# nkb-tech/nkb-classification

Measured on AMD Instinct MI355X. Metric: images/sec train step (3x224x224), higher is better.
Workload: dtype bf16; 1 GPU; resnet50 single-task train step, 1000 classes, bs=256/GPU, bf16 compute + fp32 master weights, NAdam, 3x224x224; global_batch=256, parallelism=dp1

## Files before the change

include/nkbhip.h:

```cpp
#ifndef NKBHIP_H
#define NKBHIP_H
#include <stddef.h>
#ifdef __cplusplus
extern "C" {
#endif

typedef struct ihipStream_t* nkb_stream_t;

#define NKB_DT_F32 0
#define NKB_DT_BF16 1
#define NKB_ACT_GELU 0
#define NKB_ACT_QUICK_GELU 1

const char* nkb_last_error(void);
int nkb_version(void);
enum NkbLaunchCounter {
    NKB_LAUNCH_GEMM8P = 0,
    NKB_LAUNCH_WGRAD8P = 1,
    NKB_LAUNCH_WGRAD3X3 = 2,
    NKB_LAUNCH_WGRAD8F = 3,
    NKB_LAUNCH_GRAM_CONV = 4,
    NKB_LAUNCH_GRAM_BN_APPLY = 5,
    NKB_LAUNCH_CONVP = 6,
    NKB_LAUNCH_CONV1P = 7,
// ... 81 lines not shown
                          void* g_masked, const void* c_prev, const float* scale, const float* shift, const float* mean, float* stats,
                          long long M, int Cout, int ldy, nkb_stream_t stream);
int nkb_gram_fold2(int dtype, const void* w1, const float* s1, int K1, const void* w2, const float* s2, int K2, int Cout, void* out,
                   const float* shift1, const float* shift2, float* shift_out, nkb_stream_t stream);
int nkb_conv_cat_relu_bits(int dtype, const void* a, int lda, int K1, const void* x, int ldx, int K2, const void* wf, const float* shift,
                           void* y, unsigned char* relu_bits, long long M, int Cout, int ldy, nkb_stream_t stream);
int nkb_conv_cat_bias(int dtype, const void* a, int lda, int K1, const void* x, int ldx, int K2, const void* w, const float* bias, void* y,
                      long long M, int Cout, int ldy, nkb_stream_t stream);
int nkb_conv_dgrad_bn_cat(int dtype, const void* g, int ldg, int K1, const void* a, int lda, int K2, const void* wcat,
                          const float* cbias, void* g_masked, const void* c_prev, const float* scale, const float* shift,
                          const float* mean, float* stats, long long M, int Cout, int ldy, nkb_stream_t stream);
size_t nkb_bn_backward_workspace_floats(long long rows, int C);

int nkb_maxpool3x3s2(int dtype, int backward, const void* in, void* out, unsigned char* idx, int N, int H, int W, int C,
                     nkb_stream_t stream);
enum NkbPoolMode {
    NKB_POOL_AVG_FWD = 0,
    NKB_POOL_AVG_BWD = 1,
    NKB_GRN_FWD_REDUCE = 2,
    NKB_GRN_FWD_APPLY = 3,
    NKB_GRN_BWD_REDUCE = 4,
    NKB_GRN_BWD_APPLY = 5,
    NKB_GRN_PARAM = 6
};
enum NkbSeMode {
    NKB_SE_POOL = 16,
    NKB_SE_GATE = 17,
    NKB_ECA_GATE = 18,
    NKB_SE_FWD_APPLY = 19,
    NKB_SE_BWD_REDUCE = 20,
    NKB_SE_BWD_GATE = 21,
    NKB_ECA_BWD_GATE = 22,
    NKB_SE_BWD_APPLY = 23
};
int nkb_avgpool(int dtype, int mode, const void* in, void* out, int N, int HW, int C, const void* in2, const float* weight,
                const float* bias, float* sumsq, float* dweight, float* dbias, const void* mul, float eps, float* workspace,
                long long workspace_floats, nkb_stream_t stream);
int nkb_bn_relu_maxpool(int dtype, int backward, const void* c, const float* scale, const float* shift,
                        const float* mean, const float* invstd, const float* gamma, void* y_or_g, unsigned char* idx,
                        void* dc, float* dgamma, float* dbeta, float* workspace, size_t workspace_floats, int N, int H,
                        int W, int C, nkb_stream_t stream);
int nkb_bn_relu_maxpool_sel(int dtype, int backward, const void* c, const float* scale, const float* shift,
                            const float* mean, const float* invstd, const float* gamma, void* y_or_g, unsigned char* idx,
                            void* dc, float* dgamma, float* dbeta, float* workspace, size_t workspace_floats, void* xsel,
                            int N, int H, int W, int C, nkb_stream_t stream);
size_t nkb_bn_relu_maxpool_workspace_floats(int N, int H, int W, int C);

int nkb_im2row(int dtype, const float* x, void* col, int N, int Cin, int H, int W, int R, int S, int stride, int pad,
               int Kp, nkb_stream_t stream);

int nkb_stem_pack(int dtype, const float* x, void* out, int N, int C, int H, int W, nkb_stream_t stream);
int nkb_stem_wprep(int dtype, const float* w, void* wp, int Cout, int C, nkb_stream_t stream);
int nkb_stem_weight_cols(int dtype);
int nkb_stem_conv(int dtype, const void* xp, const void* wp, void* y, float* stats, int N, int H, int W, int Cout,
                  int ldy, nkb_stream_t stream);
long long nkb_gramr_workspace_floats(int dtype, long long M, int co, int ci);
int nkb_gramr(int dtype, const void* g, int ldg, const void* a, int lda, float* R, long long M, int co, int ci, int mode,
              float* workspace, long long workspace_floats, nkb_stream_t stream);
int nkb_stemp_tiles(int dtype, int N, int H, int W, int Cout);
long long nkb_stemp_wgrad_workspace_floats(int dtype, int N, int H, int W, int Cout);
int nkb_stemp_wgrad(int dtype, const void* dy, const void* xp, float* dwp, int N, int H, int W, int Cout, int lddy, float* workspace,
                    long long workspace_floats, nkb_stream_t stream);
int nkb_stemp_conv(int dtype, const void* xp, const void* wp, void* y, float* stats, int N, int H, int W, int Cout, int ldy,
                   nkb_stream_t stream);
int nkb_stem_wgrad(int dtype, const void* dy, const void* xp, float* dwp, int N, int H, int W, int Cout, int lddy,
                   float* workspace, long long workspace_floats, nkb_stream_t stream);
// ... 133 lines not shown
```

nkb-classification_amd/csrc/conv_igemm.hip:

```cpp
#include "common.h"
#include "prims.h"
#include <type_traits>

#include "conv_params.h"
#include "wgrad256.h"
#include "gemm8p.h"
#include "wgrad3x3.h"
#include "wgradr.h"


template <typename T> struct MmaTraits;
template <> struct MmaTraits<bf16_t> { static constexpr int KSTEPS = 2; };
template <> struct MmaTraits<float> { static constexpr int KSTEPS = 8; };

constexpr int EPI_GENERAL = 0, EPI_BN_MASK = 1, EPI_BN_BITS = 2, EPI_LEAN = 3, EPI_AFFINE_BITS = 4, EPI_BN_BITS_LEAN = 6,
              EPI_BN_MASK_LEAN = 7, EPI_LEAN_CAT = 8;
template <typename T, int TC, int TP, int BNB = 0, bool HALO = false>
__global__ __launch_bounds__(256, ((BNB && TC == 128) || TC == 64) ? 3 : 1) void conv_igemm_kernel(const ConvParams p) {
    constexpr int EPC = DT<T>::EPC;
    constexpr int KTE = 128 / (int)sizeof(T);
    constexpr int NWR = TC / 32;
    constexpr int NPR = TP / 32;
    constexpr int MC = TC / 32;
    constexpr int MP = TP / 32;
    constexpr int NPX = HALO ? (TP + 2 + 31) / 32 : NPR;
    constexpr int STAGE_BYTES = (TC + 32 * NPX) * 128;
    constexpr int EROW = TC * 4 + 16;
    extern __shared__ __attribute__((aligned(16))) unsigned char smem[];

    const int tid = threadIdx.x;
    const int lane = tid & 63;
    const int wave = tid >> 6;
    const int wc = wave >> 1, wp = wave & 1;

    const unsigned nwg = gridDim.x;
// ... 1129 lines not shown
            return launch_conv_impl<T, TC, TP, BNB, true>(p, stream, batch);
    }
    return launch_conv_impl<T, TC, TP, BNB, false>(p, stream, batch);
}
static bool narrow_tile(int Cout) { return Cout <= 64; }
template <int BNB>
static int launch_conv(ConvParams& p, int dtype, bool narrow, hipStream_t stream, int batch = 1) {
    if constexpr (BNB != EPI_AFFINE_BITS && BNB != EPI_LEAN_CAT) {
        if (dtype != NKB_DT_BF16)
            return narrow ? launch_conv_tile<float, 64, 256, BNB>(p, stream, batch) : launch_conv_tile<float, 128, 128, BNB>(p, stream, batch);
    }
    if constexpr (BNB != EPI_AFFINE_BITS) {
        if (narrow) return launch_conv_tile<bf16_t, 64, 256, BNB>(p, stream, batch);
    }
    return launch_conv_tile<bf16_t, 128, 128, BNB>(p, stream, batch);
}

static ConvParams conv_geometry(int N, int H, int W, int Cin, int ldx, int P, int Q, int Cout, int ldy, int R, int S, int stride, int pad,
                                int mode) {
    ConvParams p;
    p.M = N * P * Q; p.H = H; p.W = W; p.Cin = Cin; p.ldx = ldx; p.P = P; p.Q = Q; p.Cout = Cout; p.ldy = ldy;
    p.R = R; p.S = S; p.stride = stride; p.pad = pad; p.mode = mode;
    p.stride_w = stride; p.pad_w = pad;
    p.divPQ = make_fastdiv((unsigned)(P * Q)); p.divQ = make_fastdiv((unsigned)Q);
    p.ldw = R * S * Cin;
    return p;
}
static ConvParams gemm_geometry(int M, int K, int N, int ldx, int ldw, int ldy) {
    ConvParams p = conv_geometry(1, M, 1, K, ldx, M, 1, N, ldy, 1, 1, 1, 0, 0);
    p.ldw = ldw;
    return p;
}

extern "C" int nkb_conv_gemm(int dtype, int mode, const void* x, const void* w, void* y, const void* add,
                             const float* bias, float* stats, int N, int H, int W, int Cin, int ldx, int P, int Q,
                             int Cout, int ldy, int ldadd, int R, int S, int stride, int pad, int relu, int out_f32,
                             int add_h, int add_w, const unsigned char* add_bits, hipStream_t stream) {
    const int esz = dtype == NKB_DT_BF16 ? 2 : 4;
    const int kte = 128 / esz;
    if (dtype != NKB_DT_BF16 && dtype != NKB_DT_F32) { nkb_set_error("conv_gemm: bad dtype %d", dtype); return 1; }
    if (Cin % kte != 0 || ldx % (16 / esz) != 0) {
        nkb_set_error("conv_gemm: Cin=%d must be a multiple of %d and ldx=%d of %d", Cin, kte, ldx, 16 / esz);
        return 1;
    }
    if (stride != 1 && stride != 2) { nkb_set_error("conv_gemm: stride %d unsupported", stride); return 1; }
    if (R > 32 || S > 32) { nkb_set_error("conv_gemm: %dx%d filter exceeds the 32-tap-per-axis validity masks", R, S); return 1; }
    if ((long long)N * H * W * ldx * esz >= 0xFFFFFF00ll || (long long)Cout * R * S * Cin * esz >= 0xFFFFFF00ll) {
        nkb_set_error("conv_gemm: operand exceeds the 4 GiB buffer-addressing range");
        return 1;
    }
    if ((long long)N * H * W * ldx >= (1ll << 31) || (long long)N * P * Q * ldy >= (1ll << 31) ||
        (long long)Cout * R * S * Cin >= (1ll << 31)) {
        nkb_set_error("conv_gemm: tensor exceeds 2^31 elements");
        return 1;
    }
    if (add_bits && (add == nullptr || add_h > 0 || ldadd % 8 != 0)) { nkb_set_error("conv_gemm: add_bits needs a full-grid add with ldadd %% 8 == 0"); return 1; }
    ConvParams p = conv_geometry(N, H, W, Cin, ldx, P, Q, Cout, ldy, R, S, stride, pad, mode);
    p.x = x; p.w = w; p.y = y; p.add = add; p.bias = bias; p.stats = stats;
    p.ldadd = ldadd; p.relu = relu; p.out_f32 = out_f32;
    p.add_h = add_h; p.add_w = add_w; p.add_bits = add_bits;
    const double flops = 2.0 * p.M * (double)Cout * R * S * Cin;
    const double bytes = ((double)N * H * W * Cin + (double)Cout * R * S * Cin) * esz +
                         (double)p.M * Cout * (out_f32 ? 4 : esz) * (add ? 2 : 1);
    NkbProfScope prof(mode == 0 ? NKB_K_CONV_FWD : NKB_K_CONV_DGRAD, stream, flops, bytes);
    if (nkb_gemm8p_eligible(p, dtype, 1)) return nkb_launch_gemm8p(p, stream);
    return launch_conv<EPI_GENERAL>(p, dtype, narrow_tile(Cout), stream);
}

extern "C" int nkb_conv_dgrad_bn(int dtype, const void* dy, const void* w, void* g_masked, const void* c,
                                 const float* scale, const float* shift, const float* mean, float* stats,
                                 const unsigned char* relu_bits, const void* add, int ldadd, const unsigned char* add_bits,
                                 int add_h, int add_w, int N, int H,
                                 int W, int Cin, int ldx, int P, int Q, int Cout, int ldy, int R, int S, int stride, int pad,
                                 hipStream_t stream) {
    const int esz = dtype == NKB_DT_BF16 ? 2 : 4;
    const int kte = 128 / esz;
    if (dtype != NKB_DT_BF16 && dtype != NKB_DT_F32) { nkb_set_error("conv_dgrad_bn: bad dtype %d", dtype); return 1; }
    if (Cin % kte != 0 || ldx % (16 / esz) != 0 || Cout % 8 != 0 || ldy % 8 != 0) {
        nkb_set_error("conv_dgrad_bn: Cin=%d must be a multiple of %d, Cout=%d / ldy=%d of 8", Cin, kte, Cout, ldy);
        return 1;
    }
    if (stride != 1 && stride != 2) { nkb_set_error("conv_dgrad_bn: stride %d unsupported", stride); return 1; }
    if (R > 32 || S > 32) { nkb_set_error("conv_dgrad_bn: filter too large"); return 1; }
    if ((long long)N * H * W * ldx * esz >= 0xFFFFFF00ll || (long long)Cout * R * S * Cin * esz >= 0xFFFFFF00ll ||
        (long long)N * P * Q * ldy >= (1ll << 31)) {
        nkb_set_error("conv_dgrad_bn: operand exceeds the addressing range");
        return 1;
    }
    if (relu_bits == nullptr && (add != nullptr || scale == nullptr || shift == nullptr)) {
        nkb_set_error("conv_dgrad_bn: the recomputed-mask form takes scale/shift and no residual operand");
        return 1;
    }
    if (add && ((add_h == 0 && ldadd % 8 != 0) || (add_bits && add_h > 0))) { nkb_set_error("conv_dgrad_bn: bad add operand (ldadd=%d)", ldadd); return 1; }
    ConvParams p = conv_geometry(N, H, W, Cin, ldx, P, Q, Cout, ldy, R, S, stride, pad, 1);
    p.x = dy; p.w = w; p.y = g_masked; p.add = add; p.stats = stats; p.aux = c;
    p.ldadd = ldadd; p.add_h = add_h; p.add_w = add_w; p.add_bits = add_bits;
    p.bn_bits = relu_bits; p.bn_scale = scale; p.bn_shift = shift; p.bn_mean = mean;
    NkbProfScope prof(NKB_K_CONV_DGRAD, stream, 2.0 * p.M * (double)Cout * R * S * Cin,
// ... 438 lines not shown
```

nkb-classification_amd/csrc/elementwise.hip:

```cpp
#include "common.h"
#include <stdlib.h>
#include <atomic>

static inline unsigned grid_for(size_t work_items, int block = 256, unsigned cap = 256 * 16) {
    size_t g = (work_items + block - 1) / block;
    if (g > cap) g = cap;
    if (g < 1) g = 1;
    return (unsigned)g;
}

static inline int env_int(const char* name, int dflt) {
    const char* v = getenv(name);
    return v && *v ? atoi(v) : dflt;
}
#ifndef NKB_BN_FUSED
#define NKB_BN_FUSED 1
#endif
static constexpr int g_bn_fused = NKB_BN_FUSED;

template <int NC>
__device__ __forceinline__ void ldvec(const float* __restrict__ p, float* o) {
#pragma unroll
    for (int i = 0; i < NC / 4; ++i) {
        const f32x4 v = *(const f32x4*)(p + 4 * i);
// ... 565 lines not shown
    for (size_t i = (size_t)blockIdx.x * blockDim.x + threadIdx.x; i < total; i += (size_t)gridDim.x * blockDim.x) {
        const int cg = (int)(i % cpr), n = (int)(i / cpr);
        float acc[NC];
#pragma unroll
        for (int e = 0; e < NC; ++e) acc[e] = 0.f;
        for (int k = 0; k < HW; ++k) {
            float v[NC];
            Chunk<T>::load(x + ((size_t)n * HW + k) * C + cg * NC, v);
#pragma unroll
            for (int e = 0; e < NC; ++e) acc[e] += v[e];
        }
        const float inv = 1.f / (float)HW;
#pragma unroll
        for (int e = 0; e < NC; ++e) acc[e] *= inv;
        Chunk<T>::store(y + (size_t)n * C + cg * NC, acc);
    }
}
template <typename T>
__global__ void avgpool_bwd_kernel(const T* __restrict__ g, T* __restrict__ dx, int N, int HW, int C) {
    constexpr int NC = Chunk<T>::N;
    const int cpr = C / NC;
    const size_t total = (size_t)N * HW * cpr;
    const float inv = 1.f / (float)HW;
    for (size_t i = (size_t)blockIdx.x * blockDim.x + threadIdx.x; i < total; i += (size_t)gridDim.x * blockDim.x) {
        const int cg = (int)(i % cpr);
        const int n = (int)(i / ((size_t)cpr * HW));
        float v[NC];
        Chunk<T>::load(g + (size_t)n * C + cg * NC, v);
#pragma unroll
        for (int e = 0; e < NC; ++e) v[e] *= inv;
        Chunk<T>::store(dx + i * NC, v);
    }
}
extern "C" int nkb_avgpool(int dtype, int mode, const void* in, void* out, int N, int HW, int C, const void* in2, const float* weight,
                           const float* bias, float* sumsq, float* dweight, float* dbias, const void* mul, float eps, float* workspace,
                           long long workspace_floats, hipStream_t stream) {
    if (mode >= NKB_SE_POOL && mode <= NKB_SE_BWD_APPLY)
        return nkb_se(dtype, mode, in, out, N, HW, C, in2, weight, bias, sumsq, dweight, dbias, mul, workspace, workspace_floats, stream);
    if (mode < NKB_POOL_AVG_FWD || mode > NKB_GRN_PARAM) { nkb_set_error("avgpool: bad mode %d", mode); return 1; }
    if (mode >= NKB_GRN_FWD_REDUCE)
        return nkb_grn(dtype, mode, in, out, N, HW, C, in2, weight, bias, sumsq, dweight, dbias, mul, eps, workspace, workspace_floats, stream);
    const int backward = mode;
    const int n = dtype == NKB_DT_BF16 ? 8 : 4;
    if (C % n) { nkb_set_error("avgpool: C=%d not a multiple of %d", C, n); return 1; }
    NkbProfScope prof(NKB_K_AVGPOOL, stream, 0);
    const size_t total = backward ? (size_t)N * HW * (C / n) : (size_t)N * (C / n);
    const unsigned grid = backward ? grid_for(total) : grid_for(total, 64);
    const int blk = backward ? 256 : 64;
    if (dtype == NKB_DT_BF16) {
        if (!backward) hipLaunchKernelGGL(avgpool_fwd_kernel<bf16_t>, dim3(grid), dim3(blk), 0, stream, (const bf16_t*)in, (bf16_t*)out, N, HW, C);
        else hipLaunchKernelGGL(avgpool_bwd_kernel<bf16_t>, dim3(grid), dim3(blk), 0, stream, (const bf16_t*)in, (bf16_t*)out, N, HW, C);
    } else {
        if (!backward) hipLaunchKernelGGL(avgpool_fwd_kernel<float>, dim3(grid), dim3(blk), 0, stream, (const float*)in, (float*)out, N, HW, C);
        else hipLaunchKernelGGL(avgpool_bwd_kernel<float>, dim3(grid), dim3(blk), 0, stream, (const float*)in, (float*)out, N, HW, C);
    }
    return nkb_check_launch("avgpool");
}

template <typename T>
__global__ void avgpool2x2_fwd_kernel(const T* __restrict__ x, T* __restrict__ y, int N, int H, int W, int C, int P, int Q) {
    constexpr int NC = Chunk<T>::N;
    const int cpr = C / NC;
    const size_t total = (size_t)N * P * Q * cpr;
    for (size_t i = (size_t)blockIdx.x * blockDim.x + threadIdx.x; i < total; i += (size_t)gridDim.x * blockDim.x) {
        const int cg = (int)(i % cpr);
        size_t pix = i / cpr;
        const int q = (int)(pix % Q); pix /= Q;
        const int pp = (int)(pix % P);
        const int n = (int)(pix / P);
// ... 856 lines not shown
```

nkb-classification_amd/nkb_classification/backbones.py:

```python
from __future__ import annotations

import math
from typing import List, Optional, Sequence

import torch
from torch import nn

from .hipnet import HipEngine


class _ParamOnly(nn.Module):
    def forward(self, *a, **k):
        raise RuntimeError("this module only stores parameters; it is executed by the owning HIP classifier "
                           "(call the classifier returned by get_model, on a cuda device)")


def transformer_layer_groups(backbone: nn.Module) -> List[List[nn.Parameter]]:
    depth = len(backbone.blocks)
    groups: List[List[nn.Parameter]] = [[] for _ in range(depth + 2)]
    for name, p in backbone.named_parameters():
        head = name.split(".")[0]
        if head == "blocks":
            k = int(name.split(".")[1]) + 1
        elif head in ("cls_token", "pos_embed", "patch_embed", "norm_pre"):
# ... 138 lines not shown
        return [self.conv1[0]] if self.deep_stem else [self.conv1]

    def _deep_stem_forward(self, eng: HipEngine, img: torch.Tensor, train: bool) -> torch.Tensor:
        from . import hip
        N, C, H, W = img.shape
        c0, b0, _, c1, b1, _, c2 = self.conv1
        P, Q = (H + 2 - 3) // 2 + 1, (W + 2 - 3) // 2 + 1
        kp = eng.kpad(C * 9)
        col = eng.ws.get("stem.col", (N, P, Q, kp), eng.T)
        hip.im2row(eng.d, img, col, N, C, H, W, 3, 3, 2, 1, kp)
        x = eng.conv_bn("stem0", col, c0, b0, True, None, train, col_input=True).view(N, P, Q, c0.out_channels)
        x = eng.conv_bn("stem1", x, c1, b1, True, None, train)
        return eng.conv_bn("stem", x, c2, self.bn1, True, None, train, pool=True)

    def run_forward(self, eng: HipEngine, img: torch.Tensor, train: bool) -> torch.Tensor:
        from . import hip
        N, C, H, W = img.shape
        conv = self.conv1
        if self.deep_stem:
            x = self._deep_stem_forward(eng, img, train)
        elif eng.packed_stem(conv):
            xp = eng.ws.get("stem.xp", (N, H, (W + 1) // 2 * 2, 4), eng.T)
            hip.stem_pack(eng.d, img, xp, N, C, H, W)
            x = eng.conv_bn("stem", xp, conv, self.bn1, True, None, train, pool=True, stem_packed=(N, H, W))
        else:
            R, st, pad = conv.kernel_size[0], conv.stride[0], conv.padding[0]
            P, Q = (H + 2 * pad - R) // st + 1, (W + 2 * pad - R) // st + 1
            kp = eng.kpad(C * R * R)
            col = eng.ws.get("stem.col", (N, P, Q, kp), eng.T)
            hip.im2row(eng.d, img, col, N, C, H, W, R, R, st, pad, kp)
            x = eng.conv_bn("stem", col, conv, self.bn1, True, None, train, col_input=True, pool=True)
        all_blocks = list(self.blocks())
        nblocks = len(all_blocks)
        for bi, (name, blk) in enumerate(all_blocks):
            inp = x
            stages = blk.stages()
            short, short_affine = inp, None
            se = getattr(blk, "se", None)
            want_gram = (isinstance(blk, _Bottle) and bi + 1 < nblocks and train and se is None
                         and not eng.s2_classes(all_blocks[bi + 1][1].stages()[0][0]))
            proj = None
            dpool, dconv, dbn = self.shortcut(blk) if blk.downsample is not None else (None, None, None)
            if blk.downsample is not None and dpool is None and want_gram and eng.gram_proj_ok(dconv, stages[-1][0]):
                proj = (dconv, dbn, inp, f"{name}.ds")
            elif blk.downsample is not None:
                box = {}

                def shortcut(key=f"{name}.ds", src=inp, pool=dpool, cv=dconv, bn=dbn):
                    if pool is not None:
                        src = eng.avgpool2(key + "p", src, train)
                    box["r"] = eng.conv_bn(key, src, cv, bn, False, None, train, defer_apply=True)
                eng.on_side(shortcut)
            for k, (cv, bn) in enumerate(stages[:-1]):
                x = eng.conv_bn(f"{name}.{k}", x, cv, bn, True, None, train, gram_out=want_gram and k == len(stages) - 2)
            if blk.downsample is not None and proj is None:
                eng.join_side()
                short, s_scale, s_shift = box["r"]
                short_affine = (s_scale, s_shift) if s_scale is not None else None
            cv, bn = stages[-1]
            gram = want_gram and eng.can_fuse_bn_backward(f"{name}.{len(stages) - 2}")
            if proj is not None and not gram:
                raise RuntimeError(f"{name}: projection shortcut planned into a Gram-form closing stage that did not qualify")
            if se is not None:
                x = eng.conv_bn_se(f"{name}.{len(stages) - 1}", x, cv, bn, se, short, short_affine, train)
                continue
            x = eng.conv_bn(f"{name}.{len(stages) - 1}", x, cv, bn, True, short, train, res_affine=short_affine, gram=gram, proj=proj)
        return eng.avgpool("gap", x)

    def run_backward(self, eng: HipEngine, g_emb: torch.Tensor, on_done=None):
        g = eng.avgpool_backward("gap", g_emb, "g0")
        flip = 1
        blocks = list(self.blocks())
        g_stats = None
        for bi in range(len(blocks) - 1, -1, -1):
            name, blk = blocks[bi]
            eng.begin_block(bi)
            n = len(blk.stages())
            last = f"{name}.{n - 1}"
            top = n - 1
            if eng.saved[last].get("gram") is not None:
                if g_stats is None:
                    raise RuntimeError(f"{last}: the Gram-form closing stage needs the fused residual BN-backward producer")
                prev = f"{name}.{n - 2}"
                ga, st = eng.gram_closing_backward(last, g, g_stats, prev, f"a{n - 1}")
                gc = eng.bn_backward_fused(prev, ga, st, f"c{n - 1}")
                bits = None
                top = n - 2
            elif eng.saved[last].get("se") is not None:
                assert g_stats is None
                gc = eng.se_closing_backward(last, g, "t0")
                bits = eng.saved[last]["bits"]
            elif g_stats is not None:
                gc = eng.bn_backward_fused(last, g, g_stats, "t0")
                bits = None
            else:
                gc = eng.bn_backward(last, g, "t0")
                bits = eng.saved[last]["bits"]
            for k in range(top, 0, -1):
                prev = f"{name}.{k - 1}"
# ... 101 lines not shown
```

nkb-classification_amd/nkb_classification/hip.py:

```python
from __future__ import annotations

import ctypes as C
import os
from pathlib import Path

import torch

from . import cabi

F32, BF16 = 0, 1
_TORCH_DT = {torch.float32: F32, torch.bfloat16: BF16}

_LIB = None
_LIB_PATH = Path(__file__).resolve().parents[1] / "lib" / "libnkbhip.so"

_HEADER = cabi.header_text()
_PROTOS = cabi.parse(_HEADER)
_SIGS = {name: (p.restype, p.argtypes) for name, p in _PROTOS.items()}


def lib_path() -> Path:
    return Path(os.environ.get("NKBHIP_LIB", _LIB_PATH))


# ... 474 lines not shown

def bn_backward_ws(rows, C_):
    return load().nkb_bn_backward_workspace_floats(rows, C_)


def bn_relu_maxpool(dtype, backward, c, scale, shift, mean, invstd, gamma, y_or_g, idx, dc, dgamma, dbeta, work, N, H, W, C_, xsel=None):
    check(load().nkb_bn_relu_maxpool_sel(dtype, int(backward), ptr(c), ptr(scale), ptr(shift), ptr(mean), ptr(invstd),
                                         ptr(gamma), ptr(y_or_g), ptr(idx), ptr(dc), ptr(dgamma), ptr(dbeta), ptr(work),
                                         work.numel() if work is not None else 0, ptr(xsel), N, H, W, C_, stream()), "bn_relu_maxpool")


def bn_relu_maxpool_ws(N, H, W, C_) -> int:
    return int(load().nkb_bn_relu_maxpool_workspace_floats(N, H, W, C_))


def maxpool(dtype, backward, src, dst, idx, N, H, W, C_):
    check(load().nkb_maxpool3x3s2(dtype, int(backward), ptr(src), ptr(dst), ptr(idx), N, H, W, C_, stream()), "maxpool")


_POOL_MODES = cabi.parse_enum(_HEADER, "NkbPoolMode")


def _pool(what, dtype, mode, src, dst, N, HW, C_, in2=None, weight=None, bias=None, sumsq=None, dweight=None, dbias=None, mul=None,
          eps=0.0, workspace=None):
    check(load().nkb_avgpool(dtype, _POOL_MODES[mode], ptr(src), ptr(dst), N, HW, C_, ptr(in2), ptr(weight), ptr(bias), ptr(sumsq),
                             ptr(dweight), ptr(dbias), ptr(mul), eps, ptr(workspace), workspace.numel() if workspace is not None else 0,
                             stream()), what)


def avgpool(dtype, backward, src, dst, N, HW, C_):
    _pool("avgpool", dtype, "NKB_POOL_AVG_BWD" if backward else "NKB_POOL_AVG_FWD", src, dst, N, HW, C_)


def grn_workspace(N, HW, C_) -> int:
    return 2 * N * C_ + N


def grn(dtype, u, weight, bias, out, sumsq, N, HW, C_, eps=1e-6, workspace=None):
    _pool("grn", dtype, "NKB_GRN_FWD_REDUCE", u, None, N, HW, C_, sumsq=sumsq, eps=eps)
    _pool("grn", dtype, "NKB_GRN_FWD_APPLY", u, out, N, HW, C_, weight=weight, bias=bias, sumsq=sumsq, eps=eps)


def grn_backward(dtype, g, u, weight, sumsq, out, dweight, dbias, N, HW, C_, eps=1e-6, mul=None, workspace=None):
    _pool("grn_backward", dtype, "NKB_GRN_BWD_REDUCE", g, None, N, HW, C_, in2=u, sumsq=sumsq, eps=eps, workspace=workspace)
    _pool("grn_backward", dtype, "NKB_GRN_BWD_APPLY", g, out, N, HW, C_, in2=u, weight=weight, sumsq=sumsq, mul=mul, eps=eps,
          workspace=workspace)
    if dweight is not None or dbias is not None:
        grn_param(dtype, sumsq, dweight, dbias, N, HW, C_, workspace, eps=eps)


def grn_param(dtype, sumsq, dweight, dbias, N, HW, C_, workspace, eps=1e-6):
    _pool("grn_param", dtype, "NKB_GRN_PARAM", None, None, N, HW, C_, sumsq=sumsq, dweight=dweight, dbias=dbias, eps=eps,
          workspace=workspace)


_SE_MODES = cabi.parse_enum(_HEADER, "NkbSeMode")


def se_workspace(N, C_, rd=0) -> int:
    return 6 * N * C_ + 2 * C_ + C_ // 4 + 2 * N * rd


def _se(what, dtype, mode, N, hw, C_, workspace, src=None, dst=None, in2=None, weight=None, bias=None, sumsq=None, dweight=None,
        dbias=None, mul=None):
    check(load().nkb_avgpool(dtype, _SE_MODES[mode], ptr(src), ptr(dst), N, hw, C_, ptr(in2), ptr(weight), ptr(bias), ptr(sumsq),
                             ptr(dweight), ptr(dbias), ptr(mul), 0.0, ptr(workspace), workspace.numel() if workspace is not None else 0,
# ... 386 lines not shown
```

nkb-classification_amd/nkb_classification/hipnet.py:

```python
from __future__ import annotations

import os
from typing import Dict, List, Optional

import torch
from torch import nn

from . import hip, runtime
from .runtime import ParamArena, Workspace, _round_up

_ATTN_FUSED_BWD = True
_ATTN_FUSED_DQ = True
_FP8_FUSED_QUANT = os.environ.get("NKB_FP8_FUSED_QUANT", "1") != "0"
_LN_BWD_SCALED_COPY = True
_FP8_LN_BWD_QUANT = True
_GRAM_MAX_C = 128


class HipEngine:

    def __init__(self, arena: ParamArena, device, dtype: torch.dtype):
        self.arena = arena
        self.device = device
        self.T = dtype
# ... 227 lines not shown
    @staticmethod
    def _momentum(bn) -> float:
        return bn.momentum if bn.momentum is not None else 0.1

    def _save_stage(self, key, x, conv, bn, geom, rows, bnvec, **over):
        sv = dict(x=x, c=None, y=None, mean=bnvec[2], invstd=bnvec[3], relu=False, geom=geom, conv=conv, bn=bn, rows=rows, col_input=False,
                  scale=bnvec[0], shift=bnvec[1], has_res=False, pool_idx=None, stem_packed=False, bits=None)
        sv.update(over)
        self.saved[key] = sv

    def _conv_geometry(self, w, conv, x, stem_packed, col_input):
        if w.dim() == 2:
            (co, ci), R, S, st, pad = w.shape, 1, 1, 1, 0
        else:
            co, ci, R, S = w.shape
            st, pad = conv.stride[0], conv.padding[0]
        if stem_packed:
            N, H, W = stem_packed
            P, Q = (H - 1) // 2 + 1, (W - 1) // 2 + 1
            geom = dict(N=N, H=H, W=W, Cout=co, P=P, Q=Q)
        elif col_input:
            N, P, Q, kp = x.shape
            geom = dict(N=N * P * Q, H=1, W=1, Cin=kp, ldx=kp, P=1, Q=1, Cout=co, ldy=co, R=1, S=1, stride=1, pad=0)
        else:
            N, H, W, _ = x.shape
            P, Q = (H + 2 * pad - R) // st + 1, (W + 2 * pad - S) // st + 1
            geom = dict(N=N, H=H, W=W, Cin=ci, ldx=ci, P=P, Q=Q, Cout=co, ldy=co, R=R, S=S, stride=st, pad=pad)
        narrow = not stem_packed and not col_input and self.narrow3(w, st, pad)
        return geom, N, P, Q, N * P * Q, narrow

    def conv_bn(self, key: str, x: torch.Tensor, conv: nn.Conv2d, bn: nn.BatchNorm2d, relu: bool,
                res: Optional[torch.Tensor], train: bool, col_input: bool = False, pool: bool = False,
                stem_packed=None, defer_apply: bool = False, res_affine=None, gram: bool = False, gram_out: bool = False,
                proj=None):
        w, co = conv.weight, conv.weight.shape[0]
        if w.dim() == 2:
            x = x.view(x.shape[0], 1, 1, x.shape[-1])
        geom, N, P, Q, rows, narrow = self._conv_geometry(w, conv, x, stem_packed, col_input)
        if not train and not stem_packed and not col_input and not pool:
            assert res_affine is None or res_affine[0] is None
            y = self._conv_bn_folded(key, x, w, bn, relu, res, geom, (N, P, Q), narrow)
            return (y, None, None) if defer_apply else y
        if proj is not None:
            assert gram and train and self.gram_proj_ok(proj[0], conv)
            return self._conv_bn_gram(key, x, conv, bn, None, None, geom, rows, proj=proj)
        if gram and train and self.gram_ok(conv, res, x):
            return self._conv_bn_gram(key, x, conv, bn, res, res_affine, geom, rows)
        c, stats, tiles = self._conv_raw(key, x, w, geom, (N, P, Q), narrow, train, bool(stem_packed), col_input)
        sc = self.ws.get(key + ".bnvec", (4, co), torch.float32)
        hip.bn_finalize(stats, tiles, co, rows, bn.weight, bn.bias, bn.running_mean, bn.running_var, self._momentum(bn), bn.eps, train,
                        sc[0], sc[1], sc[2], sc[3])
        if defer_apply:
            assert not relu and res is None and not pool
            if train:
                self._save_stage(key, x, conv, bn, geom, rows, sc, c=c, col_input=col_input, stem_packed=bool(stem_packed))
            return c, sc[0], sc[1]
        assert not pool or (relu and res is None)
        idx = xsel = bits = None
        if pool:
            y, idx, xsel = self._bn_pool_tail(key, c, sc, (N, P, Q), train)
        else:
            y, bits = self._bn_apply_tail(key, c, sc, relu, res, res_affine, train, gram_out)
        if train:
            self._save_stage(key, x, conv, bn, geom, rows, sc, c=c, y=y, relu=relu, col_input=col_input, has_res=res is not None,
                             pool_idx=idx, pool_xsel=xsel, stem_packed=bool(stem_packed), bits=bits)
        return y

    def _conv_bn_folded(self, key, x, w, bn, relu, res, geom, npq, narrow):
        N, P, Q = npq
        co, ci, K, rows = w.shape[0], w.shape[1], w[0].numel(), N * P * Q
        sc = self.ws.get(key + ".bnvec", (4, co), torch.float32)
        ent = self._fold.get(key)
        if ent is None or ent[0] != self.fold_key:
            hip.bn_finalize(None, 0, co, rows, bn.weight, bn.bias, bn.running_mean, bn.running_var, 0.1, bn.eps, False,
                            sc[0], sc[1], sc[2], sc[3])
            wf = ent[1] if ent is not None else runtime.empty(co, K, device=self.device, dtype=self.T)
            shift = ent[2] if ent is not None else runtime.empty(co, device=self.device, dtype=torch.float32)
            hip.wfold(self.d, self.arena.param_flat(w), sc[0], wf, co, K)
            shift.copy_(sc[1])
            ent = self._fold[key] = (self.fold_key, wf, shift)
        y = self.ws.get(key + ".y", (N, P, Q, co), self.T)
        if narrow:
            assert res is None
            H, W = geom["H"], geom["W"]
            self._stem3_tiles(N, H, W, ci, co)
            hip.stem3_conv(self.d, x, ent[1], y, N=N, H=H, W=W, Cin=ci, ldx=ci, Cout=co, ldy=co, bias=ent[2], relu=relu)
        elif w.dim() == 2 and self._splitk_ok(rows, ci, co) and res is None and not relu:
            self._splitk(key, x, ent[1], y, rows, ci, co, ent[2], None)
        else:
            hip.conv_gemm(self.d, 0, x, ent[1], y, bias=ent[2], relu=relu, add=res, ldadd=co if res is not None else 0, **geom)
        return y

    def _conv_raw(self, key, x, w, geom, npq, narrow, train, packed, col_input):
        (N, P, Q), co = npq, w.shape[0]
        rows, H, W, ci = N * P * Q, geom["H"], geom["W"], geom.get("Cin")
        c = self.ws.get(key + ".c", (N, P, Q, co), self.T)
        tiles = hip.stat_tiles(self.d, rows, co)
        tiles_p = tiles_1 = 0
        if train and self.T == torch.bfloat16 and w.dim() == 4 and not packed and not col_input:
# ... 16 lines not shown
            hip.stemp_conv(self.d, x, wf, c, stats, N, H, W, co, co)
        elif packed:
            hip.stem_conv(self.d, x, wf, c, stats, N, H, W, co, co)
        elif w.dim() == 2 and self._splitk_ok(rows, ci, co):
            self._splitk(key, x, wf, c, rows, ci, co, None, stats)
        else:
            hip.conv_gemm(self.d, 0, x, wf, c, stats=stats, **geom)
        return c, stats, tiles

    def _bn_pool_tail(self, key, c, sc, npq, train):
        (N, P, Q), co = npq, c.shape[-1]
        P2, Q2 = (P - 1) // 2 + 1, (Q - 1) // 2 + 1
        y = self.ws.get(key + ".y", (N, P2, Q2, co), self.T)
        idx = self.ws.get(key + ".idx", (N, P2, Q2, co), torch.uint8)
        xsel = self.ws.get(key + ".xsel", (N, P2, Q2, co), self.T) if train else None
        hip.bn_relu_maxpool(self.d, False, c, sc[0], sc[1], sc[2], sc[3], None, y, idx, None, None, None, None, N, P, Q, co, xsel=xsel)
        return y, idx, xsel

    def _bn_apply_tail(self, key, c, sc, relu, res, res_affine, train, gram_out):
        co, rows = c.shape[-1], c.numel() // c.shape[-1]
        y = self.ws.get(key + ".y", tuple(c.shape), self.T)
        bits = None
        if train and relu and res is not None:
            bits = self.ws.get(key + ".bits", (rows, co // (8 if self.T == torch.bfloat16 else 4)), torch.uint8)
        if gram_out and train and relu and res is None and co in (64, 128) and self.T == torch.bfloat16 and self.gram_bn:
            gs = self.ws.get(key + ".gramout", (co * co + co,), torch.float32)
            work = self.ws.at_least("gram.slabs", hip.bn_apply_gram_ws(rows, co), torch.float32)
            hip.bn_apply_gram(self.d, c, y, sc[0], sc[1], rows, co, gs, work)
            self._gram_of = (y.data_ptr(), gs)
        else:
            hip.bn_apply(self.d, c, res, y, sc[0], sc[1], rows, co, relu, bits,
                         res_scale=res_affine[0] if res_affine else None, res_shift=res_affine[1] if res_affine else None)
        return y, bits

    @staticmethod
    def _se_weights(se):
        if hasattr(se, "fc1"):
            return se.fc1.weight, se.fc1.bias, se.fc2.weight, se.fc2.bias
        return se.conv.weight, None, None, None

    def conv_bn_se(self, key: str, x: torch.Tensor, conv: nn.Conv2d, bn: nn.BatchNorm2d, se, short: torch.Tensor, res_affine, train: bool):
        c, scale, _ = self.conv_bn(key, x, conv, bn, False, None, train, defer_apply=True)
        N, P, Q, co = c.shape
        a = self.arena
        w1, b1, w2, b2 = self._se_weights(se)
        pf = lambda p: a.param_flat(p) if p is not None else None
        rd = w1.shape[0] if w2 is not None else 0
        work = self.ws.get(key + ".se", (hip.se_workspace(N, co, rd),), torch.float32)
        bnvec = self.ws.get(key + ".bnvec", (4, co), torch.float32) if scale is not None else None
        rvec = None
        if res_affine is not None:
            rvec = res_affine[0]
            assert res_affine[1].data_ptr() == rvec.data_ptr() + 4 * co
        out = self.ws.get(key + (".y" if train else ".sey"), (N, P, Q, co), self.T)
        bits = self.ws.get(key + ".bits", (N * P * Q, co // (8 if self.T == torch.bfloat16 else 4)), torch.uint8) if train else None
        w1f = pf(w1).view(rd, co) if rd else pf(w1)
        hip.se_forward(self.d, c, short, out, bnvec, work, N, P * Q, co, w1f, pf(b1), pf(w2), pf(b2), bits=bits, res_bnvec=rvec)
        if train:
            self.saved[key].update(y=out, bits=bits, has_res=True, se=dict(module=se, work=work, bnvec=bnvec))
        return out

    def se_closing_backward(self, key: str, g: torch.Tensor, slot: str) -> torch.Tensor:
        sv = self.saved[key]
        st, bn, c = sv["se"], sv["bn"], sv["c"]
        N, P, Q, co = c.shape
        a = self.arena
# ... 982 lines not shown
```

Baseline: 15310 images/sec.

## Add split-K path for small-M GEMMs and fuse final BN-apply with global avgpool

Adds a split-K path for 1x1 stride-1 GEMMs with small M (at most 256 rows) and large K. It writes fp32 partial slabs from a multi-slice launch, then sums them in a separate reduce kernel that also adds the bias. This is meant to fill CUs that a few output tiles would otherwise leave idle, for example the classifier FC at batch 256. Separately, the last bottleneck block's BN+residual+ReLU is fused with the global average pool, so the full activation tensor is never written and re-read. The cost is an extra reduce launch, a cached slab allocation, and the pool kernel's serialized per-image row loop.

```diff
diff --git a/include/nkbhip.h b/include/nkbhip.h
--- a/include/nkbhip.h
+++ b/include/nkbhip.h
@@ -137,6 +137,9 @@
     NKB_SE_BWD_GATE = 21,
     NKB_ECA_BWD_GATE = 22,
     NKB_SE_BWD_APPLY = 23
+};
+enum NkbSeamMode {
+    NKB_SEAM_APPLY_POOL = 32
 };
 int nkb_avgpool(int dtype, int mode, const void* in, void* out, int N, int HW, int C, const void* in2, const float* weight,
                 const float* bias, float* sumsq, float* dweight, float* dbias, const void* mul, float eps, float* workspace,
diff --git a/nkb-classification_amd/csrc/conv_igemm.hip b/nkb-classification_amd/csrc/conv_igemm.hip
--- a/nkb-classification_amd/csrc/conv_igemm.hip
+++ b/nkb-classification_amd/csrc/conv_igemm.hip
@@ -1,6 +1,8 @@
 #include "common.h"
 #include "prims.h"
 #include <type_traits>
+#include <map>
+#include <mutex>
 
 #include "conv_params.h"
 #include "wgrad256.h"
@@ -1196,6 +1198,95 @@
     return p;
 }
 
+#ifndef NKB_KSPLIT_MAX_M
+#define NKB_KSPLIT_MAX_M 256
+#endif
+constexpr int KSPLIT_MAX_M = NKB_KSPLIT_MAX_M, KSPLIT_MIN_K = 512, KSPLIT_MIN_KT = 4, KSPLIT_BIT = 1 << 16;
+static int gemm_ksplit(const ConvParams& p, int dtype) {
+    if (!(p.R == 1 && p.S == 1 && p.stride == 1 && p.stride_w == 1 && p.pad == 0 && p.pad_w == 0 && p.stem_cprw == 0 && p.sub_h == 0 &&
+          p.H == p.P && p.W == p.Q && p.mode == 0))
+        return 0;
+    if (p.add || p.stats || p.relu || p.act || p.add_bits || p.x2 || p.M > KSPLIT_MAX_M || p.Cin < KSPLIT_MIN_K) return 0;
+    const int kt = p.Cin / (dtype == NKB_DT_BF16 ? 64 : 32);
+    const bool narrow = p.Cout <= 64;
+    const int tiles = ((p.M + (narrow ? 255 : 127)) / (narrow ? 256 : 128)) * ((p.Cout + (narrow ? 63 : 127)) / (narrow ? 64 : 128));
+    const int cus = nkb_cu_count();
+    if (2 * tiles > cus) return 0;
+    int S = (cus + tiles - 1) / tiles;
+    if (S > kt / KSPLIT_MIN_KT) S = kt / KSPLIT_MIN_KT;
+    while (S > 1 && kt % S) --S;
+    return S >= 2 ? S : 0;
+}
+template <typename TO, int V>
+__global__ __launch_bounds__(256) void ksplit_reduce_kernel(const float* __restrict__ part, int S, int M, int N, TO* __restrict__ y, int ldy,
+                                                            const float* __restrict__ bias) {
+    const int nv = N / V;
+    const size_t i = (size_t)blockIdx.x * 256 + threadIdx.x;
+    if (i >= (size_t)M * nv) return;
+    const int m = (int)(i / nv), c = (int)(i - (size_t)m * nv) * V;
+    const float* q = part + (size_t)m * N + c;
+    const size_t slab = (size_t)M * N;
+    float v[V];
+#pragma unroll
+    for (int e = 0; e < V; ++e) v[e] = 0.f;
+    for (int z = 0; z < S; ++z) {
+        if constexpr (V == 4) {
+            const f32x4 t = *(const f32x4*)(q + (size_t)z * slab);
+            v[0] += t[0]; v[1] += t[1]; v[2] += t[2]; v[3] += t[3];
+        } else {
+            v[0] += q[(size_t)z * slab];
+        }
+    }
+#pragma unroll
+    for (int e = 0; e < V; ++e) {
+        const float o = bias ? v[e] + bias[c + e] : v[e];
+        if constexpr (sizeof(TO) == 4) y[(size_t)m * ldy + c + e] = o;
+        else y[(size_t)m * ldy + c + e] = f2bf(o);
+    }
+}
+static float* ksplit_slabs(hipStream_t stream, size_t floats) {
+    struct Slabs { float* p = nullptr; size_t floats = 0; };
+    static std::mutex mu;
+    static std::map<std::pair<int, hipStream_t>, Slabs> per_stream;
+    int dev = 0;
+    if (hipGetDevice(&dev) != hipSuccess) return nullptr;
+    std::lock_guard<std::mutex> lock(mu);
+    Slabs& s = per_stream[{dev, stream}];
+    if (s.floats < floats) {
+        if (s.p) {
+            if (hipStreamSynchronize(stream) != hipSuccess) return nullptr;
+            (void)hipFree(s.p);
+            s.p = nullptr; s.floats = 0;
+        }
+        if (hipMalloc((void**)&s.p, floats * sizeof(float)) != hipSuccess) { s.p = nullptr; return nullptr; }
+        s.floats = floats;
+    }
+    return s.p;
+}
+static int launch_gemm_ksplit(ConvParams p, int dtype, int S, hipStream_t stream) {
+    void* const y = p.y;
+    const float* const bias = p.bias;
+    const int ldy = p.ldy, out_f32 = p.out_f32 || dtype != NKB_DT_BF16, M = p.M, N = p.Cout;
+    float* slabs = ksplit_slabs(stream, (size_t)S * M * N);
+    if (!slabs) { nkb_set_error("conv_gemm: no memory for %d split-K slabs of %d x %d", S, M, N); return 1; }
+    p.Cin /= S;
+    p.sxo = p.Cin; p.swo = p.Cin; p.syo = (long long)M * N;
+    p.y = slabs; p.ldy = N; p.bias = nullptr; p.out_f32 = 1;
+    if (int rc = launch_conv<EPI_GENERAL>(p, dtype, narrow_tile(N), stream, S)) return rc;
+    g_conv_last_instance |= KSPLIT_BIT;
+    const bool v4 = (N & 3) == 0;
+    const size_t work = (size_t)M * (v4 ? N / 4 : N);
+    const dim3 grid((unsigned)((work + 255) / 256));
+    if (out_f32) {
+        if (v4) hipLaunchKernelGGL((ksplit_reduce_kernel<float, 4>), grid, dim3(256), 0, stream, slabs, S, M, N, (float*)y, ldy, bias);
+        else hipLaunchKernelGGL((ksplit_reduce_kernel<float, 1>), grid, dim3(256), 0, stream, slabs, S, M, N, (float*)y, ldy, bias);
+    } else {
+        if (v4) hipLaunchKernelGGL((ksplit_reduce_kernel<bf16_t, 4>), grid, dim3(256), 0, stream, slabs, S, M, N, (bf16_t*)y, ldy, bias);
+        else hipLaunchKernelGGL((ksplit_reduce_kernel<bf16_t, 1>), grid, dim3(256), 0, stream, slabs, S, M, N, (bf16_t*)y, ldy, bias);
+    }
+    return nkb_check_launch("conv_gemm_ksplit");
+}
+
 extern "C" int nkb_conv_gemm(int dtype, int mode, const void* x, const void* w, void* y, const void* add,
                              const float* bias, float* stats, int N, int H, int W, int Cin, int ldx, int P, int Q,
                              int Cout, int ldy, int ldadd, int R, int S, int stride, int pad, int relu, int out_f32,
@@ -1228,6 +1319,7 @@
                          (double)p.M * Cout * (out_f32 ? 4 : esz) * (add ? 2 : 1);
     NkbProfScope prof(mode == 0 ? NKB_K_CONV_FWD : NKB_K_CONV_DGRAD, stream, flops, bytes);
     if (nkb_gemm8p_eligible(p, dtype, 1)) return nkb_launch_gemm8p(p, stream);
+    if (const int S = gemm_ksplit(p, dtype)) return launch_gemm_ksplit(p, dtype, S, stream);
     return launch_conv<EPI_GENERAL>(p, dtype, narrow_tile(Cout), stream);
 }
 
diff --git a/nkb-classification_amd/csrc/elementwise.hip b/nkb-classification_amd/csrc/elementwise.hip
--- a/nkb-classification_amd/csrc/elementwise.hip
+++ b/nkb-classification_amd/csrc/elementwise.hip
@@ -621,9 +621,83 @@
         Chunk<T>::store(dx + i * NC, v);
     }
 }
+template <typename T>
+__global__ __launch_bounds__(256) void bn_apply_pool_kernel(const T* __restrict__ x, const T* __restrict__ res, const float* __restrict__ scale,
+                                                            const float* __restrict__ shift, const float* __restrict__ res_scale,
+                                                            const float* __restrict__ res_shift, unsigned char* __restrict__ bits,
+                                                            T* __restrict__ emb, int HW, int C) {
+    constexpr int N = Chunk<T>::N, CL = 32, RL = 8, W = CL * N;
+    __shared__ float tile[RL][W];
+    const int cl = threadIdx.x % CL, rl = threadIdx.x / CL;
+    const int cpr = C / N, cg = blockIdx.x * CL + cl, n = blockIdx.y;
+    const bool active = cg < cpr;
+    float sc[N], sh[N], rsc[N], rsh[N];
+    if (active) {
+        ldvec<N>(scale + cg * N, sc);
+        ldvec<N>(shift + cg * N, sh);
+        if (res_scale) { ldvec<N>(res_scale + cg * N, rsc); ldvec<N>(res_shift + cg * N, rsh); }
+    }
+    float acc = 0.f;
+    for (int k0 = 0; k0 < HW; k0 += RL) {
+        const int k = k0 + rl;
+        if (active && k < HW) {
+            const size_t row = (size_t)n * HW + k, o = row * C + (size_t)cg * N;
+            float v[N], q[N];
+            Chunk<T>::load(x + o, v);
+            if (res) Chunk<T>::load(res + o, q);
+            if (res_scale) {
+#pragma unroll
+                for (int e = 0; e < N; ++e) q[e] = DT<T>::rnd(q[e] * rsc[e] + rsh[e]);
+            }
+            unsigned b = 0u;
+#pragma unroll
+            for (int e = 0; e < N; ++e) {
+                float a = v[e] * sc[e] + sh[e];
+                if (res) a += q[e];
+                const float y = DT<T>::rnd(fmaxf(a, 0.f));
+                b |= (y > 0.f ? 1u : 0u) << e;
+                tile[rl][e * CL + cl] = y;
+            }
+            bits[row * cpr + cg] = (unsigned char)b;
+        }
+        __syncthreads();
+        if (threadIdx.x < W) {
+            const int kn = HW - k0 < RL ? HW - k0 : RL;
+            for (int j = 0; j < kn; ++j) acc += tile[j][threadIdx.x];
+        }
+        __syncthreads();
+    }
+    const int ch = blockIdx.x * W + (threadIdx.x % CL) * N + threadIdx.x / CL;
+    if (threadIdx.x < W && ch < C) DT<T>::st(emb + (size_t)n * C + ch, acc * (1.f / (float)HW));
+}
+
+static int nkb_seam_apply_pool(int dtype, const void* in, void* out, int N, int HW, int C, const void* in2, const float* bnvec,
+                               const float* bias, unsigned char* bits, hipStream_t stream) {
+    if (dtype != NKB_DT_F32 && dtype != NKB_DT_BF16) { nkb_set_error("seam: bad dtype %d", dtype); return 1; }
+    const int n = dtype == NKB_DT_BF16 ? 8 : 4, esz = dtype == NKB_DT_BF16 ? 2 : 4;
+    if (C < n || C % n) { nkb_set_error("seam: C=%d not a multiple of %d", C, n); return 1; }
+    if (N < 1 || HW < 1 || (long long)N * HW * C >= (1ll << 31) || N > 65535) {
+        nkb_set_error("seam: N=%d HW=%d C=%d outside 1 .. 2^31 elements (N up to 65535)", N, HW, C);
+        return 1;
+    }
+    if (!in || !out || !bnvec || !bits) { nkb_set_error("seam: the pass needs in, out, the BatchNorm vectors and the ReLU bits"); return 1; }
+    const double rows = (double)N * HW;
+    NkbProfScope prof(NKB_K_BN_APPLY, stream, 0, rows * C * esz * (in2 ? 2 : 1) + rows * (C / n) + (double)N * C * esz);
+    const dim3 grid((C / n + 31) / 32, N);
+    const float* rs = bias, *rb = bias ? bias + C : nullptr;
+    if (dtype == NKB_DT_BF16)
+        hipLaunchKernelGGL(bn_apply_pool_kernel<bf16_t>, grid, dim3(256), 0, stream, (const bf16_t*)in, (const bf16_t*)in2, bnvec, bnvec + C,
+                           rs, rb, bits, (bf16_t*)out, HW, C);
+    else
+        hipLaunchKernelGGL(bn_apply_pool_kernel<float>, grid, dim3(256), 0, stream, (const float*)in, (const float*)in2, bnvec, bnvec + C,
+                           rs, rb, bits, (float*)out, HW, C);
+    return nkb_check_launch("seam_apply_pool");
+}
+
 extern "C" int nkb_avgpool(int dtype, int mode, const void* in, void* out, int N, int HW, int C, const void* in2, const float* weight,
                            const float* bias, float* sumsq, float* dweight, float* dbias, const void* mul, float eps, float* workspace,
                            long long workspace_floats, hipStream_t stream) {
+    if (mode == NKB_SEAM_APPLY_POOL) return nkb_seam_apply_pool(dtype, in, out, N, HW, C, in2, weight, bias, (unsigned char*)sumsq, stream);
     if (mode >= NKB_SE_POOL && mode <= NKB_SE_BWD_APPLY)
         return nkb_se(dtype, mode, in, out, N, HW, C, in2, weight, bias, sumsq, dweight, dbias, mul, workspace, workspace_floats, stream);
     if (mode < NKB_POOL_AVG_FWD || mode > NKB_GRN_PARAM) { nkb_set_error("avgpool: bad mode %d", mode); return 1; }
diff --git a/nkb-classification_amd/nkb_classification/backbones.py b/nkb-classification_amd/nkb_classification/backbones.py
--- a/nkb-classification_amd/nkb_classification/backbones.py
+++ b/nkb-classification_amd/nkb_classification/backbones.py
@@ -194,6 +194,7 @@
             x = eng.conv_bn("stem", col, conv, self.bn1, True, None, train, col_input=True, pool=True)
         all_blocks = list(self.blocks())
         nblocks = len(all_blocks)
+        eng.saved.pop("gap", None)
         for bi, (name, blk) in enumerate(all_blocks):
             inp = x
             stages = blk.stages()
@@ -226,7 +227,11 @@
             if se is not None:
                 x = eng.conv_bn_se(f"{name}.{len(stages) - 1}", x, cv, bn, se, short, short_affine, train)
                 continue
-            x = eng.conv_bn(f"{name}.{len(stages) - 1}", x, cv, bn, True, short, train, res_affine=short_affine, gram=gram, proj=proj)
+            last = bi == nblocks - 1 and train
+            x = eng.conv_bn(f"{name}.{len(stages) - 1}", x, cv, bn, True, short, train, res_affine=short_affine, gram=gram, proj=proj,
+                            gap="gap" if last else None)
+            if "gap" in eng.saved:
+                return x
         return eng.avgpool("gap", x)
 
     def run_backward(self, eng: HipEngine, g_emb: torch.Tensor, on_done=None):
diff --git a/nkb-classification_amd/nkb_classification/hip.py b/nkb-classification_amd/nkb_classification/hip.py
--- a/nkb-classification_amd/nkb_classification/hip.py
+++ b/nkb-classification_amd/nkb_classification/hip.py
@@ -530,6 +530,14 @@
     _pool("avgpool", dtype, "NKB_POOL_AVG_BWD" if backward else "NKB_POOL_AVG_FWD", src, dst, N, HW, C_)
 
 
+_SEAM_MODES = cabi.parse_enum(_HEADER, "NkbSeamMode")
+
+
+def bn_apply_pool(dtype, c, res, emb, bnvec, bits, N, HW, C_, res_bnvec=None):
+    check(load().nkb_avgpool(dtype, _SEAM_MODES["NKB_SEAM_APPLY_POOL"], ptr(c), ptr(emb), N, HW, C_, ptr(res), ptr(bnvec), ptr(res_bnvec),
+                             ptr(bits), None, None, None, 0.0, None, 0, stream()), "bn_apply_pool")
+
+
 def grn_workspace(N, HW, C_) -> int:
     return 2 * N * C_ + N
 
diff --git a/nkb-classification_amd/nkb_classification/hipnet.py b/nkb-classification_amd/nkb_classification/hipnet.py
--- a/nkb-classification_amd/nkb_classification/hipnet.py
+++ b/nkb-classification_amd/nkb_classification/hipnet.py
@@ -283,7 +283,7 @@
     def conv_bn(self, key: str, x: torch.Tensor, conv: nn.Conv2d, bn: nn.BatchNorm2d, relu: bool,
                 res: Optional[torch.Tensor], train: bool, col_input: bool = False, pool: bool = False,
                 stem_packed=None, defer_apply: bool = False, res_affine=None, gram: bool = False, gram_out: bool = False,
-                proj=None):
+                proj=None, gap: Optional[str] = None):
         w, co = conv.weight, conv.weight.shape[0]
         if w.dim() == 2:
             x = x.view(x.shape[0], 1, 1, x.shape[-1])
@@ -308,14 +308,17 @@
             return c, sc[0], sc[1]
         assert not pool or (relu and res is None)
         idx = xsel = bits = None
+        emb = None
         if pool:
             y, idx, xsel = self._bn_pool_tail(key, c, sc, (N, P, Q), train)
+        elif gap is not None and train and relu and res is not None:
+            y, (emb, bits) = None, self._bn_apply_gap_tail(key, gap, c, sc, res, res_affine)
         else:
             y, bits = self._bn_apply_tail(key, c, sc, relu, res, res_affine, train, gram_out)
         if train:
             self._save_stage(key, x, conv, bn, geom, rows, sc, c=c, y=y, relu=relu, col_input=col_input, has_res=res is not None,
                              pool_idx=idx, pool_xsel=xsel, stem_packed=bool(stem_packed), bits=bits)
-        return y
+        return y if emb is None else emb
 
     def _conv_bn_folded(self, key, x, w, bn, relu, res, geom, npq, narrow):
         N, P, Q = npq
@@ -398,6 +401,18 @@
             hip.bn_apply(self.d, c, res, y, sc[0], sc[1], rows, co, relu, bits,
                          res_scale=res_affine[0] if res_affine else None, res_shift=res_affine[1] if res_affine else None)
         return y, bits
+
+    def _bn_apply_gap_tail(self, key, gap, c, sc, res, res_affine):
+        N, P, Q, co = c.shape
+        emb = self.ws.get(gap + ".y", (N, co), self.T)
+        bits = self.ws.get(key + ".bits", (N * P * Q, co // (8 if self.T == torch.bfloat16 else 4)), torch.uint8)
+        rvec = None
+        if res_affine is not None:
+            rvec = res_affine[0]
+            assert res_affine[1].data_ptr() == rvec.data_ptr() + 4 * co
+        hip.bn_apply_pool(self.d, c, res, emb, sc, bits, N, P * Q, co, res_bnvec=rvec)
+        self.saved[gap] = dict(in_shape=(N, P, Q, co), fused=key)
+        return emb, bits
 
     @staticmethod
     def _se_weights(se):
```

Result: no change. 15330 images/sec, median of 6 (+0.2%).
